# tky823/ssspy

Measured on AMD Instinct MI355X. Metric: GaussILRMA-IP1 update_once mixture-iterations/sec (F=1025,T=512,N=4,K=16), higher is better.
Workload: dtype f64; 1 GPU; BASELINE configs[1] GaussILRMA-IP1/MM (N=M=4, F=1025, T=512, n_basis=16) x 128 independent mixtures per GPU (configs[4] shard), record_loss=False, update_once() = one fused C-ABI call; batch_per_gpu=128, global_batch=128, n_bins=1025, n_frames=512, n_basis=16, parallelism=mixtures sharded, no collective, input=nmf_mixture(seed=1000+b) per mixture b (SURVEY 8d)

## Files before the change

### ssspy_amd/csrc/ilrma_api.hip

```cpp
#include "ilrma_plan.hpp"

namespace ssspy {

static inline int check_model(int source_model, double param, double domain = 2.0) {
  const int model = source_model & 0xff;
  const bool me = (source_model & SSSPY_SOURCE_ME) != 0;
  if ((source_model & ~(0xff | SSSPY_SOURCE_ME)) != 0)
    return fail(SSSPY_ERR_BADARG, "bad source model flags");
  if (me && (domain != 2.0 || model == SSSPY_SOURCE_GGD))
    return fail(SSSPY_ERR_BADARG, "ME source updates need domain == 2 and a Gauss or t model");
  if (model == SSSPY_SOURCE_GAUSS) return SSSPY_OK;
  if (model == SSSPY_SOURCE_T && param > 0.0) return SSSPY_OK;
  if (model == SSSPY_SOURCE_GGD && param > 0.0 && param < 2.0) return SSSPY_OK;
  return fail(SSSPY_ERR_BADARG, "bad source model / model_param (t: dof > 0, GGD: 0 < beta < 2)");
}

int ip1_with_power(void *W, const void *U, const void *C, double *qbuf, int B, int F, int N,
                   int floor_kind, double floor_eps, int *info, hipStream_t st);
int separate_power(const void *X, const void *W, double *P, int B, int N, int F, int T,
                   hipStream_t st);
int row_power(const void *W, const void *C, double *qbuf, int B, int F, int N, hipStream_t st);
int wb_update_basis(const double *a, const double *b, double *basis, const double *activation,
                    double *nd, int BN, int F, int T, int K, const IlrmaDims &d, hipStream_t st);
int wb_update_activation(const double *a, const double *b, const double *basis, double *activation,
                         double *nd, int BN, int F, int T, int K, const IlrmaDims &d,
                         hipStream_t st);
int wb_tv_weights(int mode, const double *basis, const double *activation, const double *ypow,
                  const void *y, double *out0, double *out1, int BN, int F, int T, int K,
                  const IlrmaDims &d, hipStream_t st);
int wb_loss_data(const double *basis, const double *activation, const double *ypow, const void *y,
                 double *out, void *ws, int B, int N, int F, int T, int K, const IlrmaDims &d,
                 hipStream_t st);

__global__ __launch_bounds__(256) void k_ilrma_activation_finalize(double *act,
                                                                   const double *__restrict__ part,
                                                                   int N, int K, int T,
                                                                   int nchunks, IlrmaDims d) {
  const int b = blockIdx.z, n = blockIdx.y;
  const long long e = (long long)blockIdx.x * blockDim.x + threadIdx.x;
  if (e >= (long long)K * T) return;
  double sn = 0.0, sd = 0.0;
// ... 501 lines not shown
  return check_launch("k_ilrma_activation_finalize");
}

int ssspy_ilrma_update_activation(const void *X, const void *W, const double *basis,
                                  double *activation, int B, int N, int F, int T, int K,
                                  double domain, int source_model, double model_param,
                                  int floor_kind, double floor_eps, void *workspace,
                                  size_t workspace_bytes, void *stream) {
  SSSPY_REQUIRE(X && basis && activation && B > 0 && F > 0 && T > 0,
                "update_activation: bad argument");
  SSSPY_REQUIRE(K >= 1 && K <= SSSPY_MAX_BASIS, "update_activation: n_basis must be in [1, 65536]");
  int rc = check_model(source_model, model_param, domain);
  if (rc) return rc;
  const IlrmaWs w = ilrma_ws(B, N, F, T, K);
  SSSPY_REQUIRE(workspace && workspace_bytes >= w.total, "update_activation: workspace too small");
  const IlrmaPlan p = make_ilrma_plan(B, N, F, T, K, domain, source_model, model_param);
  const IlrmaDims d = make_dims(B, F, T, K, domain, source_model, model_param, floor_kind, floor_eps);
  return activation_pass(p, w, d, X, W, false, basis, activation, (char *)workspace,
                         as_stream(stream));
}

static int wcov_into(const IlrmaPlan &p, const IlrmaWs &w, const IlrmaDims &d, const void *X,
                     const void *W, const double *basis, const double *activation, void *U,
                     char *ws, const void *Ysep, bool ysep_is_power, hipStream_t st) {
  const int N = p.N;
  double *wbuf = (double *)(ws + w.wbuf);
  const void *Y = Ysep ? Ysep : (W ? nullptr : X);
  const bool ypow = Ysep && ysep_is_power;
  const bool gauss2 = p.gauss && d.p == 2.0;
  int rc;
  switch (cov_route(p, Ysep != nullptr, W != nullptr)) {
    case CovRoute::RuntimeN:
      if (!(p.gauss || Y))
        return fail(SSSPY_ERR_UNSUPPORTED,
                    "ILRMA above 8 sources: covariance weights need the Gauss model or the separated "
                    "spectrogram");
      rc = launch_iss_weight(gauss2, Y, ypow, basis, activation, wbuf, N, d, st);
      if (rc) return rc;
      return rt_covariance(X, X, wbuf, SSSPY_WEIGHT_BIN_FRAME, U, d.B, N, N, d.F, d.T, st);
    case CovRoute::WideBasis:
      rc = wb_tv_weights(2, basis, activation, ypow ? (const double *)Y : nullptr,
                         ypow ? nullptr : Y, wbuf, nullptr, d.B * N, d.F, d.T, d.K, d, st);
      if (rc) return rc;
      return ssspy_weighted_covariance(X, wbuf, SSSPY_WEIGHT_BIN_FRAME, U, d.B, N, N, d.F, d.T, st);
    case CovRoute::MatrixCore:
      rc = launch_iss_weight(gauss2, Y, ypow, basis, activation, wbuf, N, d, st);
      if (rc) return rc;
      return wide_weighted_cov(X, wbuf, SSSPY_WEIGHT_BIN_FRAME, U, d.B, N, N, d.F, d.T, st);
    case CovRoute::Tuned:
      ILRMA_FAST_DISPATCH(N, ilrma_fast_wcov, X, W, basis, activation, U, d.B, d.F, d.T, d.K,
                          ws + w.upart, p.fm_id, p.fm_param, d.floor_kind, d.floor_eps, st, nullptr,
                          nullptr);
    default:
      ILRMA_DISPATCH(N, ilrma_wcov, X, W, basis, activation, U, d, st);
  }
}

int ssspy_ilrma_weighted_covariance(const void *X, const void *W, const double *basis,
                                    const double *activation, void *U, int B, int N, int F, int T,
                                    int K, double domain, int source_model, double model_param,
                                    int floor_kind, double floor_eps, void *workspace,
                                    size_t workspace_bytes, void *stream) {
  SSSPY_REQUIRE(X && basis && activation && U && B > 0 && F > 0 && T > 0,
                "ilrma_weighted_covariance: bad argument");
  SSSPY_REQUIRE(K >= 1 && K <= SSSPY_MAX_BASIS, "ilrma_weighted_covariance: bad n_basis");
  int rc = check_model(source_model, model_param, domain);
  if (rc) return rc;
  const IlrmaWs w = ilrma_ws(B, N, F, T, K);
  SSSPY_REQUIRE(workspace && workspace_bytes >= w.total,
                "ilrma_weighted_covariance: workspace too small");
  char *ws = (char *)workspace;
  hipStream_t st = as_stream(stream);
  const IlrmaPlan p = make_ilrma_plan(B, N, F, T, K, domain, source_model, model_param);
  const IlrmaDims d = make_dims(B, F, T, K, domain, source_model, model_param, floor_kind, floor_eps);
  const void *Ysep = nullptr;
// ... 159 lines not shown
      rc = ssspy_sum_logdet(W, logdet, B, F, N, stream);
      if (rc) return rc;
    }
  }
  const void *Xs = X, *Ws = W;
  if (p.power_once) {
    rc = separate_power(X, W, (double *)(ws + w.ybuf), B, N, F, T, st);
    if (rc) return rc;
    Xs = ws + w.ybuf;
    Ws = nullptr;
  }
  rc = check_basis_args(Xs, basis, activation, B, F, T, K, domain, source_model, model_param);
  if (rc) return rc;
  const IlrmaDims d = make_dims(B, F, T, K, domain, source_model, model_param, floor_kind, floor_eps);
  rc = basis_pass(p, w, d, Xs, Ws, p.power_once, basis, activation, ws, loss_data, loss_stride, st);
  if (rc) return rc;
  rc = activation_pass(p, w, d, Xs, Ws, p.power_once, basis, activation, ws, st);
  if (rc) return rc;
  double *qbuf = (double *)(ws + w.qbuf);
  if (p.ip1_latency) {
    int split = 0, rbins = 0;
    auto cov = [&]() -> int {
      ILRMA_FAST_DISPATCH(N, ilrma_fast_wcov, X, W, basis, activation, U, B, F, T, K, ws + w.upart,
                          p.fm_id, p.fm_param, floor_kind, floor_eps, st, &split, &rbins);
    };
    rc = cov();
    if (rc) return rc;
    auto ip1 = [&]() -> int {
      if (loss_data && loss_stride > 0) {
        ILRMA_FAST_DISPATCH(N, ilrma_small_ip1_logdet,
                            split ? (const void *)(ws + w.upart) : (const void *)U, split, rbins, 0ll,
                            normalize ? C : nullptr, W, B, F, floor_kind, floor_eps, qbuf, info,
                            logdet, loss_stride, st);
      }
      ILRMA_FAST_DISPATCH(N, ilrma_small_ip1, split ? (const void *)(ws + w.upart) : (const void *)U,
                          split, rbins, 0ll, normalize ? C : nullptr, W, B, F, floor_kind, floor_eps,
                          qbuf, info, st);
    };
    rc = ip1();
    if (rc || !normalize) return rc;
    ILRMA_FAST_DISPATCH(N, ilrma_small_norm, W, basis, qbuf, B, F, K, domain, floor_kind, floor_eps,
                        st);
  }
  rc = wcov_into(p, w, d, X, W, basis, activation, U, ws, p.power_once ? Xs : nullptr, p.power_once,
                 st);
  if (rc) return rc;
  rc = ip1_with_power(W, U, normalize ? C : nullptr, normalize ? qbuf : nullptr, B, F, N,
                      floor_kind, floor_eps, info, st);
  if (rc || !normalize) return rc;
  return launch_norm_scale(W, basis, qbuf, B, N, F, K, domain, floor_kind, floor_eps, st);
}

int ssspy_ilrma_ip1_update(const void *X, const void *C, void *W, double *basis, double *activation,
                           void *U, int B, int N, int F, int T, int K, double domain,
                           int source_model, double model_param, int normalize, int floor_kind,
                           double floor_eps, void *workspace, size_t workspace_bytes, int *info,
                           void *stream) {
  return ip1_update_impl(X, C, W, basis, activation, U, B, N, F, T, K, domain, source_model,
                         model_param, normalize, floor_kind, floor_eps, workspace, workspace_bytes,
                         info, nullptr, nullptr, stream);
}

int ssspy_ilrma_deferred_loss_supported(int N, int F, int T, int K, double domain,
                                        int source_model) {
  return make_ilrma_plan(1, N, F, T, K, domain, source_model).loss_byproduct;
}

int ssspy_ilrma_ip1_update_deferred_loss(const void *X, const void *C, void *W, double *basis,
                                         double *activation, void *U, int B, int N, int F, int T,
                                         int K, double domain, int source_model, double model_param,
                                         int normalize, int floor_kind, double floor_eps,
// ... 174 lines not shown
```

### ssspy_amd/csrc/ilrma_fast.hip

```cpp
#include <cstdlib>

#include "common.hpp"
#include "cov_core.hpp"
#include "fast_model.hpp"
#include "fast_tiles.hpp"
#include "tail_plan.hpp"

#ifndef SSSPY_N
#error "compile with -DSSSPY_N=<n_sources>"
#endif
#if SSSPY_N > 4
#error "fast path is built for n_sources <= 4"
#endif

#define SSSPY_CAT_(a, b) a##b
#define SSSPY_CAT(a, b) SSSPY_CAT_(a, b)
#define LAUNCHER(name) SSSPY_CAT(SSSPY_CAT(name, _n), SSSPY_N)

namespace ssspy {
namespace SSSPY_CAT(ilrma_fast_n, SSSPY_N) {

constexpr int N = SSSPY_N;
using fast::rcp_nr;
using fast::FastModel;
using fast::FM_GAUSS;
using fast::FM_GAUSS1;
using fast::FM_GAUSSP;
using fast::FM_GGD;
// ... 453 lines not shown

template <int G>
__device__ __forceinline__ void wc_half_store(const double (&acc)[4][WC_HALF], c128 *dst,
                                              double scale) {
  constexpr int PA[2][4][2] = {{{0, 1}, {2, 3}, {0, 0}, {0, 0}}, {{0, 2}, {0, 3}, {1, 2}, {1, 3}}};
  constexpr int NPAIR = G == 0 ? 2 : 4, P0 = G == 0 ? 4 : 0;
#pragma unroll
  for (int n = 0; n < 4; ++n) {
    c128 *d = dst + n * 16;
    if constexpr (G == 0) {
#pragma unroll
      for (int a = 0; a < 4; ++a) d[a * 4 + a] = cmake(acc[n][a] * scale, 0.0);
    }
#pragma unroll
    for (int p = 0; p < NPAIR; ++p) {
      const int a = PA[G][p][0], bb = PA[G][p][1];
      const double zx = acc[n][P0 + 2 * p], zy = acc[n][P0 + 2 * p + 1];
      d[a * 4 + bb] = cmake(zx * scale, zy * scale);
      d[bb * 4 + a] = cmake(zx * scale, -zy * scale);
    }
  }
}

template <int MODEL, int KS, bool FULL = false>
__global__ __launch_bounds__(256, KS >= 16 ? 1 : 2) void k_wcov_fast(const c128 *__restrict__ X,
                                                      const c128 *__restrict__ W,
                                                      const double *__restrict__ basis,
                                                      const double *__restrict__ act,
                                                      c128 *__restrict__ U, int F, int T, int K,
                                                      TailPlan plan, c128 *__restrict__ upart,
                                                      FastModel fm) {
  constexpr int SG = WC_SG;
  constexpr int WSTRIDE = N * N + 1;
  __shared__ __attribute__((aligned(16))) c128 xpatch[4][XPATCH];
  constexpr bool NEEDS_Y = MODEL == FM_T || MODEL == FM_GGD;
  __shared__ __attribute__((aligned(16))) c128 wlc[NEEDS_Y ? 4 * 16 * WSTRIDE : 1];
  constexpr bool SPLIT = WC_SHARE && !NEEDS_Y && MODEL != FM_GAUSSP && KS == 4;
  __shared__ __attribute__((aligned(16))) double phis[SPLIT ? WC_WB * N * 4 * 64 : 1];
  const int lane = threadIdx.x & 63, wave = threadIdx.x >> 6;
  const int c = lane & 15, q = lane >> 4;
  const BlockWork work = block_work(plan);
  const int b = work.b, nchunks = work.nchunks;
  const int g = wave % WC_NG, wb = wave / WC_NG;
  const int s0 = g * SG;
  const int i0 = (work.group * WC_WB + wb) * 16;
  const int bin = min(i0 + c, F - 1);
  const fast::XSrc<N> xsrc = fast::make_xsrc<N>(X + (long long)b * N * F * T, F, T);
// ... 114 lines not shown
          const double pw = cabs2(y);
          if (MODEL == FM_T) {
            den = fma(fm.w, den, fm.w1 * pw);
          } else {
            const double y2b = apply_floor(pow_nonneg(pw, 0.5 * (2.0 - fm.beta)), fm.floor_kind,
                                           fm.floor_eps);
            den = (2.0 / fm.beta) * y2b * pow_nonneg(den, 0.5 * fm.beta);
          }
        }
        if (MODEL == FM_GAUSS1) den = den * den;
        const double ph = MODEL == FM_GAUSSP ? pow_nonneg(den, -fm.pinv2) : rcp_nr(den);
        phi[s] = (valid && s0 + s < N) ? ph : 0.0;
      }
      if constexpr (!SPLIT) acc.add(x, phi);
    }
  }
  const double scale = 1.0 / (double)T;
  const int ob = i0 + c;
  auto out_bin = [&]() -> c128 * {
    return nchunks == 1 ? U + ((long long)b * F + ob) * (long long)(N * N * N)
                        : upart + (((long long)work.tail_idx * nchunks + work.chunk) * WC_BINS +
                                   (ob - work.group * WC_BINS)) * (long long)(N * N * N);
  };
  if constexpr (SPLIT) {
#pragma unroll
    for (int n = 0; n < 4; ++n)
#pragma unroll
      for (int e = 0; e < WC_HALF; ++e) {
        double v = hacc[n][e];
        v += __shfl_xor(v, 16, 64);
        v += __shfl_xor(v, 32, 64);
        hacc[n][e] = v;
      }
    if (ob < F && q == 0) {
      c128 *dst = out_bin();
      if (gu == 0) wc_half_store<0>(hacc, dst, scale);
      else wc_half_store<1>(hacc, dst, scale);
    }
    return;
  }
  acc.fold_q();
  if (ob < F) {
    c128 *dst = out_bin();
#pragma unroll
    for (int s = 0; s < SG; ++s) {
      const int n = s0 + s;
      if (n < N) {
        int e = 0;
#pragma unroll
        for (int a = 0; a < N; ++a) {
          const bool mine = (a & 3) == q;
          if (mine) dst[(n * N + a) * N + a] = cmake(acc.diag[s][a] * scale, 0.0);
#pragma unroll
          for (int bb = a + 1; bb < N; ++bb) {
            const c128 z = acc.off[s][e];
            if (mine) {
              dst[(n * N + a) * N + bb] = cmake(z.x * scale, z.y * scale);
              dst[(n * N + bb) * N + a] = cmake(z.x * scale, -z.y * scale);
            }
            ++e;
          }
        }
      }
    }
  }
// ... 60 lines not shown
    for (int s = 0; s < SG; ++s) {
      const int n = s0 + s;
      if (n < N) {
        int e = 0;
#pragma unroll
        for (int a = 0; a < N; ++a) {
          const bool mine = (a & 3) == q;
          if (mine) dst[(n * N + a) * N + a] = cmake(acc.diag[s][a] * scale, 0.0);
#pragma unroll
          for (int bb = a + 1; bb < N; ++bb) {
            const c128 z = acc.off[s][e];
            if (mine) {
              dst[(n * N + a) * N + bb] = cmake(z.x * scale, z.y * scale);
              dst[(n * N + bb) * N + a] = cmake(z.x * scale, -z.y * scale);
            }
            ++e;
          }
        }
      }
    }
  }
}

__global__ __launch_bounds__(256) void k_wcov_fold(c128 *__restrict__ U,
                                                   const c128 *__restrict__ upart, int F,
                                                   TailPlan plan) {
  constexpr int PER = WC_BINS * N * N * N;
  const int tail_idx = blockIdx.y;
  const int item = plan.full + tail_idx;
  const int b = item / plan.groups, group = item - b * plan.groups;
  const int e = blockIdx.x * blockDim.x + threadIdx.x;
  const int lb = e / (N * N * N);
  if (e >= PER || group * WC_BINS + lb >= F) return;
  const c128 s2 = ordered_sum(upart + (long long)tail_idx * plan.split * PER + e, (long long)PER,
                              plan.split);
  U[((long long)b * F + group * WC_BINS) * (long long)(N * N * N) + e] = s2;
}

template <int KS>
struct TStage {
  double t[(N * 16 * 4 * KS + 255) / 256];
  c128 w;
};

template <int KS>
constexpr int trow() {
  return 4 * KS + 1;
}

template <int KS, bool FULL>
__device__ __forceinline__ void tstage_load(TStage<KS> &st, const double *__restrict__ basis_b,
                                            const c128 *__restrict__ W_b, int F, int K, int i0) {
  constexpr int KR = 4 * KS;
#pragma unroll
  for (int u = 0; u < (N * 16 * KR + 255) / 256; ++u) {
    const int idx = threadIdx.x + 256 * u;
    const int k = idx % KR, bl = (idx / KR) & 15, n = idx / (16 * KR);
    const int bi = i0 + bl;
    double v = 0.0;
// ... 367 lines not shown
#undef SSSPY_ACT_LAUNCH_K
  return check_launch("k_activation_fast");
}

int LAUNCHER(ilrma_fast_loss)(const void *X, const void *W, const double *basis, const double *act,
                              double *out, void *loss_ws, int B, int F, int T, int K, int fmodel,
                              double mparam, hipStream_t st) {
  const TailPlan plan = make_tail_plan(B, (F + 63) / 64, (T + 15) / 16);
  const FastModel fm = make_fast_model(fmodel, mparam, 0);
  dim3 grid(plan.full + plan.tail * plan.split), block(256);
  const int nslots = plan.groups * (plan.split > 1 ? plan.split : 1) * 4;
  int rc = scalar_slots_begin(loss_ws, B, nslots, st);
  if (rc) return rc;
  double *slots = (double *)loss_ws;
  SSSPY_FAST_LAUNCH2(k_loss_fast, W != nullptr, (const c128 *)X, (const c128 *)W,
                     basis, act, slots, F, T, K, plan, fm, B);
  rc = check_launch("k_loss_fast");
  return rc ? rc : scalar_slots_fold(loss_ws, B, nslots, out, 0, st);
}

int LAUNCHER(ilrma_fast_wcov)(const void *X, const void *W, const double *basis, const double *act,
                              void *U, int B, int F, int T, int K, void *upart, int fmodel,
                              double mparam, int floor_kind, double floor_eps, hipStream_t st,
                              int *split_out = nullptr, int *rbins_out = nullptr) {
  if (split_out) *split_out = 0;
  if (rbins_out) *rbins_out = WC_BINS;
  const TailPlan plan =
      make_tail_plan(B, (F + WC_BINS - 1) / WC_BINS, (T + 15) / 16, K > 32 ? 256 : SLOTS,
                     K > 32 ? 256 : 1024);
  const FastModel fm = make_fast_model(fmodel, mparam, 0, floor_kind, floor_eps);
  dim3 grid(plan.full + plan.tail * plan.split), block(256);
#define SSSPY_WCOV_LAUNCH_F(M, KS_, FULL_)                                                        \
  hipLaunchKernelGGL((k_wcov_fast<M, KS_, FULL_>), grid, block, 0, st, (const c128 *)X,            \
                     (const c128 *)W, basis, act, (c128 *)U, F, T, K, plan, (c128 *)upart, fm)
#define SSSPY_WCOV_LAUNCH(M, KS_) SSSPY_WCOV_LAUNCH_F(M, KS_, false)
#define SSSPY_WCOV_LAUNCH_M(KS_)                       \
  switch (fmodel) {                                    \
    case FM_T: SSSPY_WCOV_LAUNCH(FM_T, KS_); break;    \
    case FM_GGD: SSSPY_WCOV_LAUNCH(FM_GGD, KS_); break; \
    case FM_GAUSS1: SSSPY_WCOV_LAUNCH(FM_GAUSS1, KS_); break; \
    case FM_GAUSSP: SSSPY_WCOV_LAUNCH(FM_GAUSSP, KS_); break; \
    default: SSSPY_WCOV_LAUNCH(FM_GAUSS, KS_); break;  \
  }
  if (K > 32) {
    SSSPY_WCOV_LAUNCH_M(16)
  } else if (K > 16) {
    SSSPY_WCOV_LAUNCH_M(8)
  } else if (full_tiles(K, T) && fmodel == FM_GAUSS) {
    SSSPY_WCOV_LAUNCH_F(FM_GAUSS, 4, true);
  } else {
    SSSPY_WCOV_LAUNCH_M(4)
  }
#undef SSSPY_WCOV_LAUNCH_M
#undef SSSPY_WCOV_LAUNCH
#undef SSSPY_WCOV_LAUNCH_F
  int rc = check_launch("k_wcov_fast");
  if (rc || plan.tail == 0) return rc;
  if (split_out && plan.full == 0) {
    *split_out = plan.split;
    return rc;
  }
  hipLaunchKernelGGL(k_wcov_fold, dim3((WC_BINS * N * N * N + 255) / 256, plan.tail), block, 0, st,
                     (c128 *)U, (const c128 *)upart, F, plan);
  return check_launch("k_wcov_fold");
}

int LAUNCHER(ilrma_fast_wcov_frame)(const void *X, const double *weight, void *U, int B, int F,
                                    int T, hipStream_t st) {
  static const bool disabled = std::getenv("SSSPY_AMD_NO_FAST") != nullptr;
  const int groups = (F + WC_BINS - 1) / WC_BINS;
  const long long items = (long long)B * groups;
  if (disabled || items < SLOTS || (long long)F * T * 16 >= (1ll << 32)) return -1;
  hipLaunchKernelGGL(k_wcov_frame_fast, dim3((unsigned)items), dim3(256), 0, st, (const c128 *)X,
                     weight, (c128 *)U, F, T, groups);
  return check_launch("k_wcov_frame_fast");
}

#endif

#undef SSSPY_FAST_LAUNCH2
#undef SSSPY_FAST_LAUNCH_M

}
```

### ssspy_amd/csrc/ilrma_plan.hpp

```cpp
#pragma once

#include <cstdlib>

#include "common.hpp"
#include "ilrma_params.hpp"
#include "tail_plan.hpp"
#include "wide_n.hpp"

namespace ssspy {

#define DECL_N(n)                                                                               \
  int ilrma_basis_n##n(const void *, const void *, const double *, double *, const double *,   \
                       IlrmaDims, hipStream_t);                                                \
  int ilrma_activation_n##n(const void *, const void *, const double *, const double *, double *, \
                            int, IlrmaDims, hipStream_t);                                      \
  int ilrma_wcov_n##n(const void *, const void *, const double *, const double *, void *,       \
                      IlrmaDims, hipStream_t);                                                 \
  size_t ilrma_loss_ws_bytes_n##n(int, int);                                                   \
  int ilrma_loss_n##n(const void *, const void *, const double *, const double *, double *,     \
                      void *, IlrmaDims, hipStream_t);
DECL_N(2) DECL_N(3) DECL_N(4) DECL_N(5) DECL_N(6) DECL_N(7) DECL_N(8)
#undef DECL_N

#define DECL_FAST(n)                                                                           \
  int ilrma_fast_basis_n##n(const void *, const void *, const double *, double *, const double *, \
                            int, int, int, int, int, double, double *, int, double, int,        \
                            double *, void *, int, hipStream_t, long long);                     \
  int ilrma_fast_basis_loss_slots_n##n(int, int, int);                                          \
  size_t ilrma_fast_loss_ws_bytes_n##n(int, int);                                               \
  int ilrma_fast_activation_n##n(const void *, const void *, const double *, double *,         \
                                 double *, int, int, int, int, int, int, double, int,           \
                                 hipStream_t, int *, int, int, double);                         \
  int ilrma_fast_wcov_n##n(const void *, const void *, const double *, const double *, void *, \
                           int, int, int, int, void *, int, double, int, double, hipStream_t,  \
                           int *, int *);                                                      \
  int ilrma_fast_loss_n##n(const void *, const void *, const double *, const double *, double *, \
                           void *, int, int, int, int, int, double, hipStream_t);
DECL_FAST(2) DECL_FAST(3) DECL_FAST(4)
#undef DECL_FAST

#define DECL_SMALL(n)                                                                           \
  size_t ilrma_small_scratch_n##n(int, int, int, int);                                            \
  int ilrma_small_activation_n##n(const void *, const void *, const double *, double *, int, int, \
                                  int, int, int, double, double *, int, double, int,              \
                                  hipStream_t);                                                   \
  int ilrma_small_ip1_n##n(const void *, int, int, long long, const void *, void *, int, int, int, \
                           double, double *, int *, hipStream_t);                                 \
  int ilrma_small_ip1_logdet_n##n(const void *, int, int, long long, const void *, void *, int,   \
                                  int, int, double, double *, int *, double *, long long,         \
                                  hipStream_t);                                                   \
  int ilrma_small_norm_n##n(void *, double *, const double *, int, int, int, double, int, double, \
                            hipStream_t);
DECL_SMALL(2) DECL_SMALL(3) DECL_SMALL(4)
#undef DECL_SMALL

bool wide_weighted_cov_ok(int N, int S, int F, int T, int kind);
int wide_weighted_cov(const void *A, const double *weight, int kind, void *U, int B, int N, int S,
                      int F, int T, hipStream_t st);
size_t wb_loss_ws_bytes(int B, int N, int F, int T);

#define ILRMA_FAST_DISPATCH(N_, fn, ...)             \
  switch (N_) {                                      \
    case 2: return fn##_n2(__VA_ARGS__);             \
    case 3: return fn##_n3(__VA_ARGS__);             \
    default: return fn##_n4(__VA_ARGS__);            \
  }
#define ILRMA_DISPATCH_OR(N_, otherwise, fn, ...)                                    \
  switch (N_) {                                                                      \
    case 2: return fn##_n2(__VA_ARGS__);                                             \
    case 3: return fn##_n3(__VA_ARGS__);                                             \
    case 4: return fn##_n4(__VA_ARGS__);                                             \
    case 5: return fn##_n5(__VA_ARGS__);                                             \
    case 6: return fn##_n6(__VA_ARGS__);                                             \
    case 7: return fn##_n7(__VA_ARGS__);                                             \
    case 8: return fn##_n8(__VA_ARGS__);                                             \
    default: return otherwise;                                                       \
  }
#define ILRMA_DISPATCH(N_, fn, ...)                                                               \
  ILRMA_DISPATCH_OR(N_, fail(SSSPY_ERR_UNSUPPORTED, "ILRMA: n_sources must be in [2, 8]"), fn, \
                    __VA_ARGS__)

static inline bool tuned_sources(int N) { return N >= 2 && N <= 4; }
// ... 92 lines not shown
enum class CovRoute { RuntimeN, WideBasis, MatrixCore, Tuned, Generic };

struct IlrmaPlan {
  int N, K;
  int fm_id, me;
  double fm_param;
  bool gauss;
  NmfRoute nmf;
  SourceRun runs[3];
  int nruns;
  int act_chunks;
  bool act_latency;
  bool act_in_place;
  bool basis_out_of_place;
  TailPlan basis_tail;
  LossRoute loss;
  bool loss_byproduct;
  int loss_slots, logdet_slots;
  bool runtime_n;
  bool cov_matrix_core;
  bool cov_tuned;
  bool power_once;
  bool ip1_latency;
  bool weights_buf;
  bool dense_buf;
  int summary;
};

static inline IlrmaPlan make_ilrma_plan(int B, int N, int F, int T, int K, double domain,
                                        int source_model, double model_param = 0.0) {
  IlrmaPlan p;
  p.N = N;
  p.K = K;
  p.fm_id = fast_model_id(domain, source_model);
  p.fm_param = p.fm_id == 4 ? domain : model_param;
  p.me = (source_model & SSSPY_SOURCE_ME) ? 1 : 0;
  p.gauss = (source_model & 0xff) == SSSPY_SOURCE_GAUSS;
  const bool fast = fast_path(N, F, T, K, domain, source_model);
  const bool small = small_path(B, N, F, T, K, domain, source_model);
  const bool wide = wide_basis_shape(N, K);
  p.nruns = source_runs(B, N, F, T, K, domain, source_model, p.runs);
  p.nmf = p.nruns               ? NmfRoute::Grouped
          : (fast && K <= 32)   ? NmfRoute::Tuned
          : wide                ? NmfRoute::WideBasis
                                : NmfRoute::Generic;
  const bool tuned = p.nmf == NmfRoute::Tuned;
  p.act_chunks = act_chunks(B, N, F, T, K);
  p.act_latency = small;
#ifdef SSSPY_NO_ACT_INPLACE
  p.act_in_place = false;
#else
  p.act_in_place = tuned && p.act_chunks == 1 && K <= 16;
#endif
  p.basis_out_of_place = K > 16;
  p.basis_tail = tuned ? ilrma_basis_plan(B, F, T, K) : TailPlan{0, 0, 1, 0};
  p.runtime_n = rt_sources_ok(N);
  p.loss = (fast && K <= 16)           ? LossRoute::Tuned
           : (K > 16 || p.runtime_n)   ? LossRoute::WideBasis
                                       : LossRoute::Generic;
  p.loss_byproduct = p.loss == LossRoute::Tuned && p.fm_id != 1;
  p.loss_slots = p.loss_byproduct ? tuned_basis_loss_slots(B, N, F, T) : 0;
  p.logdet_slots = p.loss_byproduct ? (small ? (F + 15) / 16 : 1) : 0;
  p.cov_matrix_core = N > 4 && wide_weighted_cov_ok(N, N, F, T, SSSPY_WEIGHT_BIN_FRAME);
  p.cov_tuned = fast;
  p.power_once = p.nmf == NmfRoute::Grouped || p.nmf == NmfRoute::WideBasis;
  p.ip1_latency = small;
  p.weights_buf = N > 4 || wide;
  p.dense_buf = wide;
  p.summary = p.runtime_n                      ? SSSPY_ROUTE_RUNTIME_N
              : p.nmf == NmfRoute::Grouped     ? SSSPY_ROUTE_GROUPED
              : small                          ? SSSPY_ROUTE_LATENCY
              : p.nmf == NmfRoute::WideBasis   ? SSSPY_ROUTE_WIDE_BASIS
              : tuned                          ? SSSPY_ROUTE_THROUGHPUT
                                               : SSSPY_ROUTE_GENERIC;
  return p;
}

static inline CovRoute cov_route(const IlrmaPlan &p, bool ysep, bool filter) {
  const bool weights_ok = p.gauss || ysep || !filter;
  if (p.runtime_n) return CovRoute::RuntimeN;
  if (p.K > 32 && weights_ok) return CovRoute::WideBasis;
  if (p.cov_matrix_core && weights_ok) return CovRoute::MatrixCore;
  if (p.cov_tuned && (p.gauss || filter)) return CovRoute::Tuned;
  return CovRoute::Generic;
}

static inline IlrmaPlan shape_plan(int B, int N, int F, int T, int K) {
  return make_ilrma_plan(B, N, F, T, K, 2.0, SSSPY_SOURCE_GAUSS);
}
// ... 56 lines not shown
```

### ssspy_amd/csrc/spatial_kernels.hip

```cpp
#include <cstdlib>

#include "common.hpp"
#include "cov_core.hpp"
#include "smallmat.hpp"
#include "wide_n.hpp"

namespace ssspy {
int ilrma_fast_wcov_frame_n2(const void *, const double *, void *, int, int, int, hipStream_t);
int ilrma_fast_wcov_frame_n3(const void *, const double *, void *, int, int, int, hipStream_t);
int ilrma_fast_wcov_frame_n4(const void *, const double *, void *, int, int, int, hipStream_t);

bool wide_weighted_cov_ok(int N, int S, int F, int T, int kind);
int wide_weighted_cov(const void *A, const double *weight, int kind, void *U, int B, int N, int S,
                      int F, int T, hipStream_t st);

thread_local char g_last_error[512] = "";

template <int N, bool POWER = false>
__global__ __launch_bounds__(256) void k_separate(const c128 *__restrict__ X,
                                                  const c128 *__restrict__ W, c128 *Y, int F,
                                                  int T) {
  const int i = blockIdx.x, b = blockIdx.y;
  const c128 *__restrict__ w = W + ((long long)b * F + i) * (N * N);
  const long long row0 = ((long long)b * N) * F + i;
  for (int j0 = 0; j0 < T; j0 += 2 * blockDim.x) {
    const int ja = j0 + threadIdx.x, jb = ja + blockDim.x;
// ... 277 lines not shown
    const double d = apply_floor(sqrt(qf), floor_kind, eps);
#pragma unroll
    for (int r = 0; r < N; ++r)
#pragma unroll
      for (int c = 0; c < N; ++c)
        if (r == n) Wm.a[r][c] = cmake(w[c].x / d, -w[c].y / d);
  }
  store_mat<N>(Wm, W + idx * (N * N));
  if (!ok && info) atomicAdd(info, 1);
  if (C && qbuf) {
    Mat<N> Cm;
    load_mat<N>(Cm, C + idx * (N * N));
#pragma unroll
    for (int n = 0; n < N; ++n) {
      c128 v[N];
#pragma unroll
      for (int m = 0; m < N; ++m) v[m] = cconj(Wm.a[n][m]);
      qbuf[idx * N + n] = quad_form<N>(v, Cm);
    }
  }
}

template <int N>
__global__ __launch_bounds__(64) void k_ip1_source_solve(c128 *W, const c128 *__restrict__ U,
                                                         double *__restrict__ denom,
                                                         long long nbins, int n, int *info) {
  const long long idx = (long long)blockIdx.x * blockDim.x + threadIdx.x;
  if (idx >= nbins) return;
  Mat<N> Wm, Un, A;
  load_mat<N>(Wm, W + idx * (N * N));
  load_mat<N>(Un, U + (idx * N + n) * (N * N));
  matmul<N>(A, Wm, Un);
  c128 w[N];
  const bool ok = solve_unit<N>(A, n, w);
  double qf = quad_form<N>(w, Un);
  qf = qf < 0.0 ? 0.0 : qf;
  denom[idx] = sqrt(qf);
#pragma unroll
  for (int c = 0; c < N; ++c) W[idx * (N * N) + n * N + c] = cconj(w[c]);
  if (!ok && info) atomicAdd(info, 1);
}

__global__ __launch_bounds__(256) void k_scale_filter_row(c128 *W, const double *__restrict__ denom,
                                                          long long nbins, int N, int n) {
  const long long e = (long long)blockIdx.x * blockDim.x + threadIdx.x;
  if (e >= nbins * N) return;
// ... 338 lines not shown
}

int ip1_with_power(void *W, const void *U, const void *C, double *qbuf, int B, int F, int N,
                   int floor_kind, double floor_eps, int *info, hipStream_t st) {
  const long long nbins = (long long)B * F;
  if (rt_sources_ok(N)) return rt_ip1(W, U, C, qbuf, B, F, N, floor_kind, floor_eps, info, st);
  if (ip1_small_shape(B, F, N))
    return ip1_from_records(W, U, 0, 0, 0, C, qbuf, B, F, N, floor_kind, floor_eps, info, st, nullptr, 0);
  dim3 grid((unsigned)((nbins + 63) / 64)), block(64);
  if (N > 4) {
    dim3 g8((unsigned)((nbins * 8 + 255) / 256)), b8(256);
    switch (N) {
      case 5: hipLaunchKernelGGL((k_ip1_rows<5, 8>), g8, b8, 0, st, (c128 *)W, (const c128 *)U, nbins, floor_kind, floor_eps, info, (const c128 *)C, qbuf); break;
      case 6: hipLaunchKernelGGL((k_ip1_rows<6, 8>), g8, b8, 0, st, (c128 *)W, (const c128 *)U, nbins, floor_kind, floor_eps, info, (const c128 *)C, qbuf); break;
      case 7: hipLaunchKernelGGL((k_ip1_rows<7, 8>), g8, b8, 0, st, (c128 *)W, (const c128 *)U, nbins, floor_kind, floor_eps, info, (const c128 *)C, qbuf); break;
      case 8: hipLaunchKernelGGL((k_ip1_rows<8, 8>), g8, b8, 0, st, (c128 *)W, (const c128 *)U, nbins, floor_kind, floor_eps, info, (const c128 *)C, qbuf); break;
      default: return fail(SSSPY_ERR_UNSUPPORTED, "n_sources must be in [1, 8]");
    }
    return check_launch("k_ip1_rows");
  }
  DISPATCH_N4(N, hipLaunchKernelGGL((k_ip1<NN>), grid, block, 0, st, (c128 *)W, (const c128 *)U,
                                    nbins, floor_kind, floor_eps, info, (const c128 *)C, qbuf));
  return check_launch("k_ip1");
}

int separate_power(const void *X, const void *W, double *P, int B, int N, int F, int T,
                   hipStream_t st) {
  if (rt_sources_ok(N)) return rt_separate(X, W, P, B, N, F, T, true, st);
  dim3 grid(F, B), block(256);
  DISPATCH_N(N, hipLaunchKernelGGL((k_separate<NN, true>), grid, block, 0, st, (const c128 *)X,
                                   (const c128 *)W, (c128 *)P, F, T));
  return check_launch("k_separate_power");
}

int row_power(const void *W, const void *C, double *qbuf, int B, int F, int N, hipStream_t st) {
  if (rt_sources_ok(N)) return rt_row_power(W, C, qbuf, B, F, N, st);
  const long long nbins = (long long)B * F;
  dim3 grid((unsigned)((nbins + 63) / 64)), block(64);
  DISPATCH_N(N, hipLaunchKernelGGL((k_row_power<NN>), grid, block, 0, st, (const c128 *)W,
                                   (const c128 *)C, qbuf, nbins));
  return check_launch("k_row_power");
}
}

extern "C" {

// ... 254 lines not shown
```

Baseline: 41560 iterations/s.

## Store weighted covariances in packed Hermitian planar layout for IP1 update

The weighted-covariance kernel can now write only the upper triangle of each Hermitian covariance, as separate real planes laid out bin-contiguous (structure-of-arrays), which halves the record size. A new IP1 kernel reads this packed layout with coalesced per-plane loads and stages the demixing matrices through LDS for coalesced load and store. The fold kernel for split tails gets a matching packed variant. This targets the memory traffic between the covariance and IP1 stages, at the cost of more template instantiations and a second code path that is gated by the plan and the floor kind.

```diff
diff --git a/ssspy_amd/csrc/ilrma_api.hip b/ssspy_amd/csrc/ilrma_api.hip
--- a/ssspy_amd/csrc/ilrma_api.hip
+++ b/ssspy_amd/csrc/ilrma_api.hip
@@ -17,6 +17,8 @@
 
 int ip1_with_power(void *W, const void *U, const void *C, double *qbuf, int B, int F, int N,
                    int floor_kind, double floor_eps, int *info, hipStream_t st);
+int ip1_packed_with_power(void *W, const void *P, const void *C, double *qbuf, int B, int F, int N,
+                          int floor_kind, double floor_eps, int *info, hipStream_t st);
 int separate_power(const void *X, const void *W, double *P, int B, int N, int F, int T,
                    hipStream_t st);
 int row_power(const void *W, const void *C, double *qbuf, int B, int F, int N, hipStream_t st);
@@ -564,7 +566,8 @@
 
 static int wcov_into(const IlrmaPlan &p, const IlrmaWs &w, const IlrmaDims &d, const void *X,
                      const void *W, const double *basis, const double *activation, void *U,
-                     char *ws, const void *Ysep, bool ysep_is_power, hipStream_t st) {
+                     char *ws, const void *Ysep, bool ysep_is_power, hipStream_t st,
+                     bool packed = false) {
   const int N = p.N;
   double *wbuf = (double *)(ws + w.wbuf);
   const void *Y = Ysep ? Ysep : (W ? nullptr : X);
@@ -592,7 +595,7 @@
     case CovRoute::Tuned:
       ILRMA_FAST_DISPATCH(N, ilrma_fast_wcov, X, W, basis, activation, U, d.B, d.F, d.T, d.K,
                           ws + w.upart, p.fm_id, p.fm_param, d.floor_kind, d.floor_eps, st, nullptr,
-                          nullptr);
+                          nullptr, packed ? 1 : 0);
     default:
       ILRMA_DISPATCH(N, ilrma_wcov, X, W, basis, activation, U, d, st);
   }
@@ -798,7 +801,7 @@
     int split = 0, rbins = 0;
     auto cov = [&]() -> int {
       ILRMA_FAST_DISPATCH(N, ilrma_fast_wcov, X, W, basis, activation, U, B, F, T, K, ws + w.upart,
-                          p.fm_id, p.fm_param, floor_kind, floor_eps, st, &split, &rbins);
+                          p.fm_id, p.fm_param, floor_kind, floor_eps, st, &split, &rbins, 0);
     };
     rc = cov();
     if (rc) return rc;
@@ -818,11 +821,16 @@
     ILRMA_FAST_DISPATCH(N, ilrma_small_norm, W, basis, qbuf, B, F, K, domain, floor_kind, floor_eps,
                         st);
   }
+  const bool packed = p.ip1_packed && cov_route(p, false, true) == CovRoute::Tuned &&
+                      (floor_kind == SSSPY_FLOOR_NONE || floor_kind == SSSPY_FLOOR_MAX ||
+                       floor_kind == SSSPY_FLOOR_ADD);
   rc = wcov_into(p, w, d, X, W, basis, activation, U, ws, p.power_once ? Xs : nullptr, p.power_once,
-                 st);
-  if (rc) return rc;
-  rc = ip1_with_power(W, U, normalize ? C : nullptr, normalize ? qbuf : nullptr, B, F, N,
-                      floor_kind, floor_eps, info, st);
+                 st, packed);
+  if (rc) return rc;
+  rc = packed ? ip1_packed_with_power(W, U, normalize ? C : nullptr, normalize ? qbuf : nullptr, B,
+                                      F, N, floor_kind, floor_eps, info, st)
+              : ip1_with_power(W, U, normalize ? C : nullptr, normalize ? qbuf : nullptr, B, F, N,
+                               floor_kind, floor_eps, info, st);
   if (rc || !normalize) return rc;
   return launch_norm_scale(W, basis, qbuf, B, N, F, K, domain, floor_kind, floor_eps, st);
 }
diff --git a/ssspy_amd/csrc/ilrma_fast.hip b/ssspy_amd/csrc/ilrma_fast.hip
--- a/ssspy_amd/csrc/ilrma_fast.hip
+++ b/ssspy_amd/csrc/ilrma_fast.hip
@@ -4,6 +4,7 @@
 #include "cov_core.hpp"
 #include "fast_model.hpp"
 #include "fast_tiles.hpp"
+#include "ip1_record.hpp"
 #include "tail_plan.hpp"
 
 #ifndef SSSPY_N
@@ -503,7 +504,28 @@
   }
 }
 
-template <int MODEL, int KS, bool FULL = false>
+template <int G>
+__device__ __forceinline__ void wc_half_store_packed(const double (&acc)[4][WC_HALF], double *dst,
+                                                     long long ps, double scale) {
+  constexpr int PA[2][4][2] = {{{0, 1}, {2, 3}, {0, 0}, {0, 0}}, {{0, 2}, {0, 3}, {1, 2}, {1, 3}}};
+  constexpr int NPAIR = G == 0 ? 2 : 4, P0 = G == 0 ? 4 : 0;
+#pragma unroll
+  for (int n = 0; n < 4; ++n) {
+    double *d = dst + n * ip1rec::planes(4) * ps;
+    if constexpr (G == 0) {
+#pragma unroll
+      for (int a = 0; a < 4; ++a) d[ip1rec::diag_plane(a) * ps] = acc[n][a] * scale;
+    }
+#pragma unroll
+    for (int p = 0; p < NPAIR; ++p) {
+      const int e = ip1rec::upper_index(4, PA[G][p][0], PA[G][p][1]);
+      d[ip1rec::re_plane(4, e) * ps] = acc[n][P0 + 2 * p] * scale;
+      d[ip1rec::im_plane(4, e) * ps] = acc[n][P0 + 2 * p + 1] * scale;
+    }
+  }
+}
+
+template <int MODEL, int KS, bool FULL = false, bool PACKED = false>
 __global__ __launch_bounds__(256, KS >= 16 ? 1 : 2) void k_wcov_fast(const c128 *__restrict__ X,
                                                       const c128 *__restrict__ W,
                                                       const double *__restrict__ basis,
@@ -664,6 +686,14 @@
                         : upart + (((long long)work.tail_idx * nchunks + work.chunk) * WC_BINS +
                                    (ob - work.group * WC_BINS)) * (long long)(N * N * N);
   };
+  const long long pstride = nchunks == 1 ? (long long)F : (long long)WC_BINS;
+  auto out_plane = [&]() -> double * {
+    return nchunks == 1
+               ? (double *)U + ip1rec::plane_offset(b, 0, N, 0, F) + ob
+               : (double *)upart + ((long long)work.tail_idx * nchunks + work.chunk) *
+                                       (long long)(WC_BINS * N * N * N) +
+                     (ob - work.group * WC_BINS);
+  };
   if constexpr (SPLIT) {
 #pragma unroll
     for (int n = 0; n < 4; ++n)
@@ -675,14 +705,46 @@
         hacc[n][e] = v;
       }
     if (ob < F && q == 0) {
-      c128 *dst = out_bin();
-      if (gu == 0) wc_half_store<0>(hacc, dst, scale);
-      else wc_half_store<1>(hacc, dst, scale);
+      if constexpr (PACKED) {
+        double *dst = out_plane();
+        if (gu == 0) wc_half_store_packed<0>(hacc, dst, pstride, scale);
+        else wc_half_store_packed<1>(hacc, dst, pstride, scale);
+      } else {
+        c128 *dst = out_bin();
+        if (gu == 0) wc_half_store<0>(hacc, dst, scale);
+        else wc_half_store<1>(hacc, dst, scale);
+      }
     }
     return;
   }
   acc.fold_q();
   if (ob < F) {
+    if constexpr (PACKED) {
+      double *dst = out_plane();
+#pragma unroll
+      for (int s = 0; s < SG; ++s) {
+        const int n = s0 + s;
+        if (n < N) {
+          double *d = dst + n * ip1rec::planes(N) * pstride;
+          int e = 0;
+#pragma unroll
+          for (int a = 0; a < N; ++a) {
+            const bool mine = (a & 3) == q;
+            if (mine) d[ip1rec::diag_plane(a) * pstride] = acc.diag[s][a] * scale;
+#pragma unroll
+            for (int bb = a + 1; bb < N; ++bb) {
+              const c128 z = acc.off[s][e];
+              if (mine) {
+                d[ip1rec::re_plane(N, e) * pstride] = z.x * scale;
+                d[ip1rec::im_plane(N, e) * pstride] = z.y * scale;
+              }
+              ++e;
+            }
+          }
+        }
+      }
+      return;
+    }
     c128 *dst = out_bin();
 #pragma unroll
     for (int s = 0; s < SG; ++s) {
@@ -789,6 +851,7 @@
   }
 }
 
+template <bool PACKED>
 __global__ __launch_bounds__(256) void k_wcov_fold(c128 *__restrict__ U,
                                                    const c128 *__restrict__ upart, int F,
                                                    TailPlan plan) {
@@ -797,11 +860,20 @@
   const int item = plan.full + tail_idx;
   const int b = item / plan.groups, group = item - b * plan.groups;
   const int e = blockIdx.x * blockDim.x + threadIdx.x;
-  const int lb = e / (N * N * N);
-  if (e >= PER || group * WC_BINS + lb >= F) return;
-  const c128 s2 = ordered_sum(upart + (long long)tail_idx * plan.split * PER + e, (long long)PER,
-                              plan.split);
-  U[((long long)b * F + group * WC_BINS) * (long long)(N * N * N) + e] = s2;
+  if constexpr (PACKED) {
+    const int plane = e / WC_BINS, lb = e - plane * WC_BINS;
+    if (e >= PER || group * WC_BINS + lb >= F) return;
+    const double s2 = ordered_sum((const double *)upart + (long long)tail_idx * plan.split * PER + e,
+                                  (long long)PER, plan.split);
+    ((double *)U)[ip1rec::plane_offset(b, 0, N, 0, F) + (long long)plane * F + group * WC_BINS + lb] =
+        s2;
+  } else {
+    const int lb = e / (N * N * N);
+    if (e >= PER || group * WC_BINS + lb >= F) return;
+    const c128 s2 = ordered_sum(upart + (long long)tail_idx * plan.split * PER + e, (long long)PER,
+                                plan.split);
+    U[((long long)b * F + group * WC_BINS) * (long long)(N * N * N) + e] = s2;
+  }
 }
 
 template <int KS>
@@ -1215,34 +1287,36 @@
 int LAUNCHER(ilrma_fast_wcov)(const void *X, const void *W, const double *basis, const double *act,
                               void *U, int B, int F, int T, int K, void *upart, int fmodel,
                               double mparam, int floor_kind, double floor_eps, hipStream_t st,
-                              int *split_out = nullptr, int *rbins_out = nullptr) {
+                              int *split_out, int *rbins_out, int packed) {
   if (split_out) *split_out = 0;
   if (rbins_out) *rbins_out = WC_BINS;
+  if (packed && (K > 32 || split_out))
+    return fail(SSSPY_ERR_INTERNAL, "ilrma_fast_wcov: no packed form for this call");
   const TailPlan plan =
       make_tail_plan(B, (F + WC_BINS - 1) / WC_BINS, (T + 15) / 16, K > 32 ? 256 : SLOTS,
                      K > 32 ? 256 : 1024);
   const FastModel fm = make_fast_model(fmodel, mparam, 0, floor_kind, floor_eps);
   dim3 grid(plan.full + plan.tail * plan.split), block(256);
-#define SSSPY_WCOV_LAUNCH_F(M, KS_, FULL_)                                                        \
-  hipLaunchKernelGGL((k_wcov_fast<M, KS_, FULL_>), grid, block, 0, st, (const c128 *)X,            \
+#define SSSPY_WCOV_LAUNCH_F(M, KS_, FULL_, PACKED_)                                               \
+  hipLaunchKernelGGL((k_wcov_fast<M, KS_, FULL_, PACKED_>), grid, block, 0, st, (const c128 *)X,   \
                      (const c128 *)W, basis, act, (c128 *)U, F, T, K, plan, (c128 *)upart, fm)
-#define SSSPY_WCOV_LAUNCH(M, KS_) SSSPY_WCOV_LAUNCH_F(M, KS_, false)
-#define SSSPY_WCOV_LAUNCH_M(KS_)                       \
-  switch (fmodel) {                                    \
-    case FM_T: SSSPY_WCOV_LAUNCH(FM_T, KS_); break;    \
-    case FM_GGD: SSSPY_WCOV_LAUNCH(FM_GGD, KS_); break; \
-    case FM_GAUSS1: SSSPY_WCOV_LAUNCH(FM_GAUSS1, KS_); break; \
-    case FM_GAUSSP: SSSPY_WCOV_LAUNCH(FM_GAUSSP, KS_); break; \
-    default: SSSPY_WCOV_LAUNCH(FM_GAUSS, KS_); break;  \
+#define SSSPY_WCOV_LAUNCH(M, KS_, PACKED_) SSSPY_WCOV_LAUNCH_F(M, KS_, false, PACKED_)
+#define SSSPY_WCOV_LAUNCH_M(KS_, PACKED_)                       \
+  switch (fmodel) {                                             \
+    case FM_T: SSSPY_WCOV_LAUNCH(FM_T, KS_, PACKED_); break;    \
+    case FM_GGD: SSSPY_WCOV_LAUNCH(FM_GGD, KS_, PACKED_); break; \
+    case FM_GAUSS1: SSSPY_WCOV_LAUNCH(FM_GAUSS1, KS_, PACKED_); break; \
+    case FM_GAUSSP: SSSPY_WCOV_LAUNCH(FM_GAUSSP, KS_, PACKED_); break; \
+    default: SSSPY_WCOV_LAUNCH(FM_GAUSS, KS_, PACKED_); break;  \
   }
   if (K > 32) {
-    SSSPY_WCOV_LAUNCH_M(16)
+    SSSPY_WCOV_LAUNCH_M(16, false)
   } else if (K > 16) {
-    SSSPY_WCOV_LAUNCH_M(8)
+    if (packed) { SSSPY_WCOV_LAUNCH_M(8, true) } else { SSSPY_WCOV_LAUNCH_M(8, false) }
   } else if (full_tiles(K, T) && fmodel == FM_GAUSS) {
-    SSSPY_WCOV_LAUNCH_F(FM_GAUSS, 4, true);
+    if (packed) { SSSPY_WCOV_LAUNCH_F(FM_GAUSS, 4, true, true); } else { SSSPY_WCOV_LAUNCH_F(FM_GAUSS, 4, true, false); }
   } else {
-    SSSPY_WCOV_LAUNCH_M(4)
+    if (packed) { SSSPY_WCOV_LAUNCH_M(4, true) } else { SSSPY_WCOV_LAUNCH_M(4, false) }
   }
 #undef SSSPY_WCOV_LAUNCH_M
 #undef SSSPY_WCOV_LAUNCH
@@ -1253,8 +1327,11 @@
     *split_out = plan.split;
     return rc;
   }
-  hipLaunchKernelGGL(k_wcov_fold, dim3((WC_BINS * N * N * N + 255) / 256, plan.tail), block, 0, st,
-                     (c128 *)U, (const c128 *)upart, F, plan);
+  const dim3 fgrid((WC_BINS * N * N * N + 255) / 256, plan.tail);
+  if (packed)
+    hipLaunchKernelGGL(k_wcov_fold<true>, fgrid, block, 0, st, (c128 *)U, (const c128 *)upart, F, plan);
+  else
+    hipLaunchKernelGGL(k_wcov_fold<false>, fgrid, block, 0, st, (c128 *)U, (const c128 *)upart, F, plan);
   return check_launch("k_wcov_fold");
 }
 
diff --git a/ssspy_amd/csrc/ilrma_plan.hpp b/ssspy_amd/csrc/ilrma_plan.hpp
--- a/ssspy_amd/csrc/ilrma_plan.hpp
+++ b/ssspy_amd/csrc/ilrma_plan.hpp
@@ -33,7 +33,7 @@
                                  hipStream_t, int *, int, int, double);                         \
   int ilrma_fast_wcov_n##n(const void *, const void *, const double *, const double *, void *, \
                            int, int, int, int, void *, int, double, int, double, hipStream_t,  \
-                           int *, int *);                                                      \
+                           int *, int *, int);                                                 \
   int ilrma_fast_loss_n##n(const void *, const void *, const double *, const double *, double *, \
                            void *, int, int, int, int, int, double, hipStream_t);
 DECL_FAST(2) DECL_FAST(3) DECL_FAST(4)
@@ -58,6 +58,7 @@
 int wide_weighted_cov(const void *A, const double *weight, int kind, void *U, int B, int N, int S,
                       int F, int T, hipStream_t st);
 size_t wb_loss_ws_bytes(int B, int N, int F, int T);
+bool ip1_small_shape(int B, int F, int N);
 
 #define ILRMA_FAST_DISPATCH(N_, fn, ...)             \
   switch (N_) {                                      \
@@ -196,6 +197,7 @@
   bool cov_tuned;
   bool power_once;
   bool ip1_latency;
+  bool ip1_packed;
   bool weights_buf;
   bool dense_buf;
   int summary;
@@ -239,6 +241,11 @@
   p.cov_tuned = fast;
   p.power_once = p.nmf == NmfRoute::Grouped || p.nmf == NmfRoute::WideBasis;
   p.ip1_latency = small;
+#ifdef SSSPY_NO_PACKED_IP1
+  p.ip1_packed = false;
+#else
+  p.ip1_packed = tuned && !small && !ip1_small_shape(B, F, N);
+#endif
   p.weights_buf = N > 4 || wide;
   p.dense_buf = wide;
   p.summary = p.runtime_n                      ? SSSPY_ROUTE_RUNTIME_N
diff --git a/ssspy_amd/csrc/ip1_record.hpp b/ssspy_amd/csrc/ip1_record.hpp
--- /dev/null
+++ b/ssspy_amd/csrc/ip1_record.hpp
@@ -0,0 +1,37 @@
+#pragma once
+
+namespace ssspy {
+namespace ip1rec {
+
+constexpr int pairs(int N) { return (N * (N - 1)) / 2; }
+constexpr int planes(int N) { return N * N; }
+constexpr int upper_index(int N, int a, int b) { return a * N - (a * (a + 1)) / 2 + (b - a - 1); }
+constexpr int diag_plane(int a) { return a; }
+constexpr int re_plane(int N, int e) { return N + e; }
+constexpr int im_plane(int N, int e) { return N + pairs(N) + e; }
+constexpr long long plane_offset(long long b, int n, int N, int plane, long long F) {
+  return ((b * N + n) * planes(N) + plane) * F;
+}
+
+constexpr bool layout_ok(int N) {
+  int e = 0;
+  for (int a = 0; a < N; ++a)
+    for (int b = a + 1; b < N; ++b) {
+      if (upper_index(N, a, b) != e) return false;
+      ++e;
+    }
+  if (e != pairs(N)) return false;
+  int next = 0;
+  for (int a = 0; a < N; ++a)
+    if (diag_plane(a) != next++) return false;
+  for (int k = 0; k < pairs(N); ++k)
+    if (re_plane(N, k) != next++) return false;
+  for (int k = 0; k < pairs(N); ++k)
+    if (im_plane(N, k) != next++) return false;
+  return next == planes(N);
+}
+static_assert(layout_ok(2) && layout_ok(3) && layout_ok(4), "packed IP1 record layout");
+static_assert(planes(4) * sizeof(double) * 2 == 16 * 16, "half of the full-layout record");
+
+}
+}
diff --git a/ssspy_amd/csrc/spatial_kernels.hip b/ssspy_amd/csrc/spatial_kernels.hip
--- a/ssspy_amd/csrc/spatial_kernels.hip
+++ b/ssspy_amd/csrc/spatial_kernels.hip
@@ -2,6 +2,7 @@
 
 #include "common.hpp"
 #include "cov_core.hpp"
+#include "ip1_record.hpp"
 #include "smallmat.hpp"
 #include "wide_n.hpp"
 
@@ -325,6 +326,112 @@
 }
 
 template <int N>
+__device__ __forceinline__ void ip1_rows_to_lds(c128 *lds, const c128 *__restrict__ g, int count,
+                                                int lane) {
+  constexpr int NN = N * N;
+#pragma unroll
+  for (int t = 0; t < NN; ++t) {
+    const int i = t * 64 + lane;
+    if (i < count) lds[(i / NN) * (NN + 1) + (i % NN)] = g[i];
+  }
+}
+template <int N>
+__device__ __forceinline__ void ip1_rows_from_lds(const c128 *lds, c128 *g, int count, int lane) {
+  constexpr int NN = N * N;
+#pragma unroll
+  for (int t = 0; t < NN; ++t) {
+    const int i = t * 64 + lane;
+    if (i < count) g[i] = lds[(i / NN) * (NN + 1) + (i % NN)];
+  }
+}
+
+template <int N>
+__global__ __launch_bounds__(64) void k_ip1_packed(c128 *W, const double *__restrict__ P,
+                                                   long long nbins, int F, int floor_kind,
+                                                   double eps, int *info,
+                                                   const c128 *__restrict__ C, double *qbuf) {
+  constexpr int NN = N * N;
+  __shared__ __attribute__((aligned(16))) c128 patch[64 * (NN + 1)];
+  const int lane = threadIdx.x;
+  const long long base = (long long)blockIdx.x * 64;
+  const long long idx = base + lane;
+  const bool live = idx < nbins;
+  const int rows = (int)(nbins - base < 64 ? nbins - base : 64);
+  const c128 *mine = patch + lane * (NN + 1);
+  ip1_rows_to_lds<N>(patch, W + base * NN, rows * NN, lane);
+  __syncthreads();
+  Mat<N> Wm;
+  bool ok = true;
+  if (live) {
+    load_mat<N>(Wm, mine);
+    const long long b = idx / F, f = idx - b * F;
+    const double *Pb = P + ip1rec::plane_offset(b, 0, N, 0, F) + f;
+#pragma unroll 1
+    for (int n = 0; n < N; ++n) {
+      const double *Pn = Pb + (long long)n * NN * F;
+      Mat<N> Un, A;
+#pragma unroll
+      for (int a = 0; a < N; ++a) Un.a[a][a] = cmake(Pn[(long long)ip1rec::diag_plane(a) * F], 0.0);
+#pragma unroll
+      for (int a = 0; a < N; ++a)
+#pragma unroll
+        for (int bb = a + 1; bb < N; ++bb) {
+          const int e = ip1rec::upper_index(N, a, bb);
+          const double re = Pn[(long long)ip1rec::re_plane(N, e) * F];
+          const double im = Pn[(long long)ip1rec::im_plane(N, e) * F];
+          Un.a[a][bb] = cmake(re, im);
+          Un.a[bb][a] = cmake(re, -im);
+        }
+      matmul<N>(A, Wm, Un);
+      c128 w[N];
+      ok = solve_unit<N>(A, n, w) && ok;
+      double qf = quad_form<N>(w, Un);
+      qf = qf < 0.0 ? 0.0 : qf;
+      const double d = apply_floor(sqrt(qf), floor_kind, eps);
+#pragma unroll
+      for (int r = 0; r < N; ++r)
+#pragma unroll
+        for (int c = 0; c < N; ++c)
+          if (r == n) Wm.a[r][c] = cmake(w[c].x / d, -w[c].y / d);
+    }
+  }
+  __syncthreads();
+  if (live) store_mat<N>(Wm, patch + lane * (NN + 1));
+  __syncthreads();
+  ip1_rows_from_lds<N>(patch, W + base * NN, rows * NN, lane);
+  if (!ok && info) atomicAdd(info, 1);
+  if (C && qbuf) {
+    __syncthreads();
+    ip1_rows_to_lds<N>(patch, C + base * NN, rows * NN, lane);
+    __syncthreads();
+    double q[N];
+    if (live) {
+      Mat<N> Cm;
+      load_mat<N>(Cm, mine);
+#pragma unroll
+      for (int n = 0; n < N; ++n) {
+        c128 v[N];
+#pragma unroll
+        for (int m = 0; m < N; ++m) v[m] = cconj(Wm.a[n][m]);
+        q[n] = quad_form<N>(v, Cm);
+      }
+    }
+    __syncthreads();
+    double *qp = (double *)patch;
+    if (live) {
+#pragma unroll
+      for (int n = 0; n < N; ++n) qp[lane * (N + 1) + n] = q[n];
+    }
+    __syncthreads();
+#pragma unroll
+    for (int t = 0; t < N; ++t) {
+      const int i = t * 64 + lane;
+      if (i < rows * N) qbuf[base * N + i] = qp[(i / N) * (N + 1) + (i % N)];
+    }
+  }
+}
+
+template <int N>
 __global__ __launch_bounds__(64) void k_ip1_source_solve(c128 *W, const c128 *__restrict__ U,
                                                          double *__restrict__ denom,
                                                          long long nbins, int n, int *info) {
@@ -709,6 +816,19 @@
   DISPATCH_N4(N, hipLaunchKernelGGL((k_ip1<NN>), grid, block, 0, st, (c128 *)W, (const c128 *)U,
                                     nbins, floor_kind, floor_eps, info, (const c128 *)C, qbuf));
   return check_launch("k_ip1");
+}
+
+int ip1_packed_with_power(void *W, const void *P, const void *C, double *qbuf, int B, int F, int N,
+                          int floor_kind, double floor_eps, int *info, hipStream_t st) {
+  const long long nbins = (long long)B * F;
+  dim3 grid((unsigned)((nbins + 63) / 64)), block(64);
+  switch (N) {
+    case 2: hipLaunchKernelGGL((k_ip1_packed<2>), grid, block, 0, st, (c128 *)W, (const double *)P, nbins, F, floor_kind, floor_eps, info, (const c128 *)C, qbuf); break;
+    case 3: hipLaunchKernelGGL((k_ip1_packed<3>), grid, block, 0, st, (c128 *)W, (const double *)P, nbins, F, floor_kind, floor_eps, info, (const c128 *)C, qbuf); break;
+    case 4: hipLaunchKernelGGL((k_ip1_packed<4>), grid, block, 0, st, (c128 *)W, (const double *)P, nbins, F, floor_kind, floor_eps, info, (const c128 *)C, qbuf); break;
+    default: return fail(SSSPY_ERR_INTERNAL, "ip1_packed_with_power: shape off the packed path");
+  }
+  return check_launch("k_ip1_packed");
 }
 
 int separate_power(const void *X, const void *W, double *P, int B, int N, int F, int T,
```

After: 41940 iterations/s, median of 6. No clear change (+0.9%).
